# phylo42/EPIK

Measured on AMD Instinct MI355X. Metric: reads placed/sec, higher is better.
Workload: dtype f32

## Files before the change

epik_amd/capi.py:

```python
from __future__ import annotations

import ctypes
import os

import numpy as np

_HERE = os.path.dirname(os.path.abspath(__file__))
LIB_PATH = os.environ.get("EPIK_AMD_LIB") or os.path.join(_HERE, "libepik_amd.so")

ABI_VERSION = 3

OK, ERR_INVALID, ERR_NO_DEVICE, ERR_HIP, ERR_UNSUPPORTED = 0, 1, 2, 3, 4

PLACEMENT = np.dtype([("branch", np.uint32), ("score", np.float32), ("lwr", np.float64)])
CONFIDENCE = np.dtype([("clade", np.uint32), ("clade_mass_q", np.uint32), ("edpl", np.float64)])
TAXON_RECORD = np.dtype([("taxon", np.uint32), ("taxon_mass_q", np.uint32), ("first_taxon", np.uint32), ("total_q", np.uint32)])
WINDOW_RECORD = np.dtype([("call", np.uint32), ("call_mass_q", np.uint32), ("first_group", np.uint32), ("total_q", np.uint32)])
WINDOW_SEGMENT = np.dtype([("call", np.uint32), ("first_window", np.uint32), ("num_windows", np.uint32), ("reserved", np.uint32),
                           ("call_mass", np.uint64), ("total", np.uint64)])
TAXA_TOTALS = np.dtype([(name, np.uint64) for name in ("placed", "no_hit", "too_short", "too_narrow", "no_mass", "bad_reads")])
SQUASH_MERGE = np.dtype([("a", np.uint32), ("b", np.uint32), ("dist", np.float64), ("len_a", np.float64), ("len_b", np.float64)])
SQUASH_NONE = 0xFFFFFFFF
EPCA_INFO = np.dtype([("used", np.uint32), ("components", np.uint32), ("sweeps", np.uint32), ("converged", np.uint32),
                      ("trace", np.float64), ("scale", np.float64)])
# ... 71 lines not shown
RAREFY_MAX_DEPTHS = 256
RAREFY_MAX_DEPTH = 1 << 20
PKDB_VALUE = np.dtype([("branch", np.uint32), ("score", np.float32)])

EXPORTS = (
    "epik_amd_device_count",
    "epik_amd_last_error",
    "epik_amd_placer_create",
    "epik_amd_placer_plan",
    "epik_amd_placer_plan_sizes",
    "epik_amd_placer_build_image",
    "epik_amd_placer_plan_run_counts",
    "epik_amd_placer_run_counts",
    "epik_amd_placer_ring_form",
    "epik_amd_placer_table_form",
    "epik_amd_placer_destroy",
    "epik_amd_placer_place",
    "epik_amd_placer_place_device",
    "epik_amd_placer_algorithmic_bytes",
    "epik_amd_placer_create_sharded",
    "epik_amd_placer_accumulate_device",
    "epik_amd_placer_finish_device",
    "epik_amd_placer_partial_info",
    "epik_amd_placer_accumulate_lists_device",
    "epik_amd_placer_finish_lists_device",
    "epik_amd_placer_last_path",
    "epik_amd_placer_stream_build",
    "epik_amd_placer_place_sharded",
    "epik_amd_placer_release_scratch",
    "epik_amd_placer_set_wide_counts",
# ... 263 lines not shown
    0xFFFFFFFF, 0xFFFFFFFE, 0xFFFFFFFD, 0xFFFFFFFC, 0xFFFFFFFB, 0xFFFFFFFA)
WINDOW_CLASSES = {WINDOW_TOO_NARROW: "too_narrow", WINDOW_TOO_SHORT: "too_short", WINDOW_NO_HIT: "no_hit",
                  WINDOW_BAD_ROW: "bad_row", WINDOW_NO_MASS: "no_mass", WINDOW_AMBIGUOUS: "ambiguous"}

STRAND_FORWARD, STRAND_REVERSE, STRAND_BOTH = 0, 1, 2
STRANDS = {"forward": STRAND_FORWARD, "reverse": STRAND_REVERSE, "both": STRAND_BOTH}

MATES_FF = 0x100
MATE_ORIENTATIONS = {"fr": 0, "ff": MATES_FF}

FRAMES_FORWARD, FRAMES_REVERSE, FRAMES_BOTH = 0, 1, 2
FRAME_MODES = {"forward": FRAMES_FORWARD, "reverse": FRAMES_REVERSE, "both": FRAMES_BOTH}
FRAME_NAMES = ("+1", "+2", "+3", "-1", "-2", "-3")

ROWS_COUNTS_TOO_NARROW = 0xFFFFFFFF


class EpikAmdError(RuntimeError):
    def __init__(self, code: int, message: str):
        super().__init__(f"libepik_amd error {code}: {message}")
        self.code = code


_lib = None


def hip_runtimes(maps_text: str | None = None) -> list:
    import re
    if maps_text is None:
        try:
# ... 62 lines not shown
    lib.epik_amd_placer_plan_sizes.restype = i32
    lib.epik_amd_placer_plan_sizes.argtypes = [ctypes.c_uint32] * 4 + [ctypes.POINTER(ListBin), u64, ctypes.c_uint32, ctypes.c_uint32,
                                               u64, ctypes.POINTER(Plan)]
    lib.epik_amd_placer_build_image.restype = i32
    lib.epik_amd_placer_build_image.argtypes = [ctypes.POINTER(PlacerDesc), ctypes.c_uint32, ctypes.c_uint32, u64,
                                                vp, vp, vp]
    lib.epik_amd_placer_plan_run_counts.restype = i32
    lib.epik_amd_placer_plan_run_counts.argtypes = [ctypes.POINTER(PlacerDesc), ctypes.c_uint32, ctypes.c_uint32, u64,
                                                    ctypes.c_uint32, ctypes.POINTER(ctypes.c_uint32)]
    lib.epik_amd_placer_run_counts.restype = i32
    lib.epik_amd_placer_run_counts.argtypes = [vp, ctypes.c_uint32, ctypes.POINTER(ctypes.c_uint32)]
    lib.epik_amd_placer_ring_form.restype = i32
    lib.epik_amd_placer_ring_form.argtypes = [vp, ctypes.c_uint32, ctypes.POINTER(ctypes.c_uint32)]
    lib.epik_amd_placer_table_form.restype = i32
    lib.epik_amd_placer_table_form.argtypes = [vp, ctypes.POINTER(ctypes.c_uint32)]
    lib.epik_amd_placer_destroy.restype = None
    lib.epik_amd_placer_destroy.argtypes = [vp]
    lib.epik_amd_placer_place.restype = i32
    lib.epik_amd_placer_place.argtypes = [vp, vp, vp, u64, vp, vp, vp]
    lib.epik_amd_placer_place_device.restype = i32
    lib.epik_amd_placer_place_device.argtypes = [vp, vp, vp, u64, vp, vp, vp, vp]
    lib.epik_amd_placer_algorithmic_bytes.restype = i32
    lib.epik_amd_placer_algorithmic_bytes.argtypes = [vp, vp, vp, u64, vp, vp, ctypes.POINTER(u64)]
    lib.epik_amd_placer_launch_info.restype = i32
    lib.epik_amd_placer_launch_info.argtypes = [vp, ctypes.POINTER(ctypes.c_uint32),
                                                ctypes.POINTER(ctypes.c_uint32),
                                                ctypes.POINTER(ctypes.c_uint32)]
    lib.epik_amd_placer_set_wide_counts.restype = i32
    lib.epik_amd_placer_set_wide_counts.argtypes = [vp, i32]
    lib.epik_amd_placer_choose_counts.restype = i32
# ... 296 lines not shown
```

epik_amd/csrc/capi.hip:

```cpp
#include <hip/hip_runtime.h>

#include <algorithm>
#include <atomic>
#include <cmath>
#include <cstdio>
#include <cstdlib>
#include <cstring>
#include <new>
#include <string>
#include <thread>
#include <vector>

#include "db_image.hpp"
#include "epik_amd.h"
#include "place_kernel.h"
#include "placer_impl.hpp"

namespace {

thread_local std::string g_last_error;

int fail(int code, const std::string &msg)
{
    g_last_error = msg;
// ... 95 lines not shown
        (void)hipFree(p->params.dbg);
    }
#endif
    (void)hipFree(p->d_table);
    (void)hipFree(p->d_filter);
    (void)hipFree(p->d_postings);
    (void)hipFree(p->d_char_class);
    (void)hipFree(p->d_seqs);
    (void)hipFree(p->d_seq_offsets);
    (void)hipFree(p->d_rows);
    (void)hipFree(p->d_n_rows);
    (void)hipFree(p->d_counts);
    (void)hipFree(p->d_total);
    (void)hipFree(p->d_front_hdr);
    (void)hipFree(p->d_finish_hdr);
    (void)hipFree(p->d_slow_list);
    (void)hipFree(p->d_slice_rows);
    (void)hipFree(p->d_slice_sums);
    (void)hipFree(p->d_front_pool);
    (void)hipFree(p->d_front_cursor);
    (void)hipFree(p->d_sparse_cap);
    (void)hipFree(p->d_scan_tiles);
    if (p->h_front_cursor) (void)hipHostFree(p->h_front_cursor);
    if (p->ev_start) (void)hipEventDestroy(p->ev_start);
    if (p->ev_stop) (void)hipEventDestroy(p->ev_stop);
    for (hipEvent_t e : p->ev_in) (void)hipEventDestroy(e);
    for (hipEvent_t e : p->ev_kernel) (void)hipEventDestroy(e);
    if (p->stream) (void)hipStreamDestroy(p->stream);
    if (p->stream_in) (void)hipStreamDestroy(p->stream_in);
    if (p->stream_out) (void)hipStreamDestroy(p->stream_out);
// ... 143 lines not shown
    CREATE_TRY(hipMemGetInfo(&free_mem, &total_mem));
    const image::Source src{d, shard_index, shard_count};
    image::Plan &plan = p->plan;
    if (const int rc = image::make_plan(src, free_mem, std::getenv("EPIK_AMD_LAYOUT"), std::getenv("EPIK_AMD_KERNEL"),
                                        plan, err);
        rc != EPIK_AMD_OK) {
        return fail(rc, err);
    }
    p->layout = plan.layout;
    p->team = plan.layout == epik_amd::DbLayout::kTeam;
    const bool run_lists = image::run_counts_apply(plan, std::getenv("EPIK_AMD_RUN_COUNTS"));
    p->runs = run_lists ? epik_amd::kRunLists : plan.runs ? epik_amd::kRunsMixed : 0;
    {
        const char *form = std::getenv("EPIK_AMD_RING_FORM");
        p->ring_near = p->runs != 0 && plan.posting_bytes < epik_amd::kNearRegionBytes && !(form && std::strcmp(form, "far") == 0);
    }
    p->db_bytes = plan.posting_bytes;
    CREATE_TRY(hipStreamCreateWithFlags(&p->stream, hipStreamNonBlocking));
    CREATE_TRY(hipStreamCreateWithFlags(&p->stream_in, hipStreamNonBlocking));
    CREATE_TRY(hipStreamCreateWithFlags(&p->stream_out, hipStreamNonBlocking));
    CREATE_TRY(hipMalloc(&p->d_table, plan.table_bytes));
    if (plan.filter_bytes) CREATE_TRY(hipMalloc(reinterpret_cast<void **>(&p->d_filter), plan.filter_bytes));
    CREATE_TRY(hipMalloc(reinterpret_cast<void **>(&p->d_postings), plan.posting_bytes));
    {
        DeviceSink table, filter, postings;
        CREATE_TRY(table.init(static_cast<uint8_t *>(p->d_table), plan.table_bytes, p->stream_in));
        if (plan.filter_bytes)
            CREATE_TRY(filter.init(reinterpret_cast<uint8_t *>(p->d_filter), plan.filter_bytes, p->stream_out));
        CREATE_TRY(postings.init(p->d_postings, plan.posting_bytes, p->stream));
        const int rc = image::build(src, plan, table, plan.filter_bytes ? &filter : nullptr, postings, err);
// ... 25 lines not shown
    pp.filter_rec_bytes = plan.filter_rec_bytes;
    pp.entry_len_bits = plan.len_bits;
    pp.entry_cell_bits = plan.cell_bits;
    pp.postings = p->d_postings;
    pp.char_class = p->d_char_class;
    pp.sigma_pow_km1 = (uint32_t)(d->num_keys / d->alphabet_size);
    pp.kmer_size = d->kmer_size;
    pp.alphabet_size = d->alphabet_size;
    pp.num_branches = d->num_branches;
    pp.keep_at_most = d->keep_at_most;
    pp.keep_factor = d->keep_factor;
    pp.threshold = d->threshold;
    pp.log_threshold = d->log_threshold;
#ifdef EPIK_AMD_ABLATION
    if (const char *ab = std::getenv("EPIK_AMD_ABLATE")) pp.ablate = (uint32_t)std::atoi(ab);
    if (const char *e = std::getenv("EPIK_AMD_GRID_PERCENT")) p->grid_percent = std::strtoull(e, nullptr, 10);
    if (const char *st = std::getenv("EPIK_AMD_STAMPS"); st && st[0] == '1') {
        CREATE_TRY(hipMalloc(reinterpret_cast<void **>(&pp.dbg), kDbgWords * sizeof(unsigned long long)));
        CREATE_TRY(hipMemset(pp.dbg, 0, kDbgWords * sizeof(unsigned long long)));
    }
#endif
    hipDeviceProp_t prop;
    CREATE_TRY(hipGetDeviceProperties(&prop, d->device));
    if (p->team) {
        p->team_waves = plan.team_waves;
        p->team_table = static_cast<const uint8_t *>(p->d_table);
        p->team_passes = plan.team_passes;
        p->team_slice_rows = plan.team_slice_rows;
        p->team_rows_pad = plan.team_rows_pad;
        const uint32_t desc_bytes = epik_amd::team_desc_bytes(d->keep_at_most);
// ... 74 lines not shown
            const int runs = p->runs | g.ring;
            if (counts == epik_amd::kCounts8 && (pp.n_pad + 7u) / 8u > desc_bytes) {
                g.max_blocks = 0;
                continue;
            }
            if (g.lds_wave_bytes > kMaxLdsPerBlock) {
                return fail(EPIK_AMD_ERR_UNSUPPORTED, "num_branches too large for the one-wavefront-per-read kernel");
            }
            uint32_t best_waves = 0;
            for (uint32_t wpb = 4; wpb >= 1; wpb >>= 1) {
                const uint32_t block_bytes = wpb * g.lds_wave_bytes;
                if (block_bytes > kMaxLdsPerBlock) continue;
                CREATE_TRY(epik_amd::set_place_reads_lds_limit(p->layout, runs, counts, block_bytes));
                int per_cu = 0;
                CREATE_TRY(epik_amd::place_reads_occupancy(p->layout, runs, counts, (int)(wpb * 64u), block_bytes, &per_cu));
                const uint32_t lds_units = (block_bytes + epik_amd::kLdsGranule - 1u) / epik_amd::kLdsGranule;
                per_cu = std::min<int>(per_cu, (int)(128u / std::max(lds_units, 1u)));
                if (per_cu < 1) per_cu = 1;
                if ((uint32_t)per_cu * wpb > best_waves) {
                    best_waves = (uint32_t)per_cu * wpb;
                    g.waves_per_block = wpb;
                    g.lds_block_bytes = block_bytes;
                    g.max_blocks = (uint32_t)prop.multiProcessorCount * (uint32_t)per_cu;
                }
            }
            g.resident_waves = best_waves;
            CREATE_TRY(epik_amd::set_place_reads_lds_limit(p->layout, runs, counts, g.lds_block_bytes));
            CREATE_TRY(epik_amd::set_finish_reads_lds_limit(counts, g.lds_block_bytes));
        }
    }
// ... 258 lines not shown
            if (asked > est) est = asked;
        }
        want = (uint64_t)est + 1024u;
        size_t free_b = 0, total_b = 0;
        if (hipMemGetInfo(&free_b, &total_b) == hipSuccess) {
            const uint64_t room = ((uint64_t)free_b + p->front_pool_cap * 8u) / 2u / 8u;
            want = std::min<uint64_t>(want, std::max<uint64_t>(room, 1024u));
        }
    }
    want = (want + 7u) & ~7ull;
    if (want > p->front_pool_cap || (p->front_pool_forced && want != p->front_pool_cap)) {
        (void)hipFree(p->d_front_pool);
        p->d_front_pool = nullptr, p->front_pool_cap = 0;
        HIP_TRY(hipMalloc(reinterpret_cast<void **>(&p->d_front_pool), (size_t)want * sizeof(uint64_t)));
        p->front_pool_cap = want;
    }
    return EPIK_AMD_OK;
}

static int launch(epik_amd_placer *p, launch_mode mode, const void *d_seqs, const void *d_seq_offsets, uint64_t n,
                  void *d_rows, void *d_n_rows, void *d_counts, hipStream_t stream, const shard_buffers &shard = {},
                  uint64_t total_chars = 0)
{
    if (n == 0) return EPIK_AMD_OK;
    const bool lists = mode == kAccumulateLists || mode == kFinishLists;
    epik_amd::PlaceParams pp = p->params;
    pp.partial_scores = shard.scores;
    pp.partial_counts = shard.counts;
    pp.max_kmers_cap = (mode == kAccumulate || mode == kFinish) ? 65535u : 0u;
    pp.amb_slot = shard.amb_slot;
// ... 104 lines not shown
                tp.read_list = p->d_slow_list;
                tp.read_list_count = p->d_front_cursor + 1;
                HIP_TRY(epik_amd::launch_team(tp, p->team_waves, p->counts, (int)mode, dim3((unsigned)blocks),
                                              g.lds_block_bytes, stream));
                HIP_TRY(hipMemcpyAsync(p->h_front_cursor, p->d_front_cursor, 3 * sizeof(unsigned long long),
                                       hipMemcpyDeviceToHost, stream));
            }
        } else {
            HIP_TRY(epik_amd::launch_team(tp, p->team_waves, p->counts, (int)mode, dim3((unsigned)blocks), g.lds_block_bytes,
                                          stream));
        }
    } else if (mode == kFinish) {
        HIP_TRY(epik_amd::launch_finish_reads(pp, p->counts, dim3((unsigned)blocks), dim3(g.waves_per_block * 64u),
                                              g.lds_block_bytes, stream));
    } else {
        HIP_TRY(epik_amd::launch_place_reads(pp, p->layout, p->runs | p->geo[p->counts].ring, p->counts, dim3((unsigned)blocks),
                                             dim3(g.waves_per_block * 64u), g.lds_block_bytes, stream));
    }
    if (timed) {
        HIP_TRY(hipEventRecord(p->ev_stop, stream));
        p->ev_recorded = true;
    }
    return EPIK_AMD_OK;
}

int epik_amd_placer_accumulate_device(epik_amd_placer *p, const void *d_seqs, const void *d_seq_offsets,
                                      uint64_t n, void *d_scores, void *d_counts, const void *d_amb_slot,
                                      void *d_amb_order, void *d_amb_avg, void *stream)
{
    if (!p) return fail(EPIK_AMD_ERR_INVALID, "null placer");
    if (n && (!d_seqs || !d_seq_offsets || !d_scores || !d_counts))
        return fail(EPIK_AMD_ERR_INVALID, "null device buffer");
// ... 120 lines not shown

int epik_amd_placer_run_counts(const epik_amd_placer *p, uint32_t counts, uint32_t *lists)
{
    if (!p || !lists) return fail(EPIK_AMD_ERR_INVALID, "null argument");
    if (counts > (uint32_t)epik_amd::kCounts32) return fail(EPIK_AMD_ERR_INVALID, "counts must be 0, 1 or 2");
    *lists = !p->team && p->runs == epik_amd::kRunLists && counts != (uint32_t)epik_amd::kCounts8;
    return EPIK_AMD_OK;
}

int epik_amd_placer_ring_form(const epik_amd_placer *p, uint32_t counts, uint32_t *form)
{
    if (!p || !form) return fail(EPIK_AMD_ERR_INVALID, "null argument");
    if (counts > (uint32_t)epik_amd::kCounts32) return fail(EPIK_AMD_ERR_INVALID, "counts must be 0, 1 or 2");
    const int ring = p->team ? 0 : p->geo[counts].ring;
    *form = ((ring & epik_amd::kRingNear) ? EPIK_AMD_RING_NEAR : 0u) | ((ring & epik_amd::kRingSlack) ? EPIK_AMD_RING_SLACK : 0u);
    return EPIK_AMD_OK;
}

int epik_amd_placer_table_form(const epik_amd_placer *p, uint32_t *form)
{
    if (!p || !form) return fail(EPIK_AMD_ERR_INVALID, "null argument");
    switch (p->layout) {
        case epik_amd::DbLayout::kPacked:
        case epik_amd::DbLayout::kFiltered: *form = EPIK_AMD_TABLE_BY_CODE; break;
        case epik_amd::DbLayout::kPaired: *form = EPIK_AMD_TABLE_PAIRED; break;
        case epik_amd::DbLayout::kTripled: *form = EPIK_AMD_TABLE_TRIPLED; break;
        default: *form = 0u;
    }
    return EPIK_AMD_OK;
}
// ... 213 lines not shown
    return EPIK_AMD_OK;
}

int epik_amd_placer_release_scratch(epik_amd_placer *p)
{
    if (!p) return fail(EPIK_AMD_ERR_INVALID, "null placer");
    HIP_TRY(hipSetDevice(p->device));
    HIP_TRY(hipDeviceSynchronize());
    if (p->shard_state && p->shard_state_free) p->shard_state_free(p->shard_state);
    p->shard_state = nullptr;
    void **bufs[] = {reinterpret_cast<void **>(&p->d_front_hdr), reinterpret_cast<void **>(&p->d_finish_hdr),
                     reinterpret_cast<void **>(&p->d_slow_list), &p->d_slice_rows,
                     &p->d_slice_sums, reinterpret_cast<void **>(&p->d_front_pool), reinterpret_cast<void **>(&p->d_sparse_cap),
                     reinterpret_cast<void **>(&p->d_scan_tiles), reinterpret_cast<void **>(&p->d_seqs),
                     reinterpret_cast<void **>(&p->d_seq_offsets), reinterpret_cast<void **>(&p->d_rows),
                     reinterpret_cast<void **>(&p->d_n_rows), reinterpret_cast<void **>(&p->d_counts)};
    for (void **b : bufs) {
        if (*b) (void)hipFree(*b);
        *b = nullptr;
    }
    p->front_hdr_bytes = 0, p->finish_hdr_bytes = 0, p->slow_list_reads = 0, p->slice_out_reads = 0, p->front_pool_cap = 0, p->sparse_cap_items = 0;
    p->d_seqs_cap = 0, p->d_reads_cap = 0, p->front_failed_reads = 0;
    return EPIK_AMD_OK;
}

int epik_amd_placer_launch_info(const epik_amd_placer *p, uint32_t *waves_per_block,
                                uint32_t *blocks, uint32_t *lds_bytes)
{
    if (!p) return fail(EPIK_AMD_ERR_INVALID, "null placer");
    const auto &g = p->geo[p->last_geo];
    const bool streaming = p->team && p->team_front && p->last_streamed;
    if (waves_per_block) *waves_per_block = streaming ? (uint32_t)g.stream_bw[g.last_stream] : g.waves_per_block;
    if (blocks) *blocks = p->last_blocks ? p->last_blocks : streaming ? g.stream_blocks[g.last_stream] : g.max_blocks;
    if (lds_bytes) *lds_bytes = streaming ? g.stream_lds_bytes[g.last_stream] : g.lds_block_bytes;
    return EPIK_AMD_OK;
}

// ... 39 lines not shown
```

epik_amd/csrc/place_device.hpp:

```cpp
#ifndef EPIK_AMD_PLACE_DEVICE_HPP
#define EPIK_AMD_PLACE_DEVICE_HPP
#include <hip/hip_runtime.h>
#include <float.h>
#include <stdint.h>

#include <type_traits>

#include "place_kernel.h"

namespace epik_amd {

namespace {

constexpr int kWave = 64;
constexpr int kTilesPerPass = EPIK_AMD_TILES_PER_PASS;
constexpr int kRing = EPIK_AMD_RING;
static_assert((kRing & (kRing - 1)) == 0 && kRing >= 4 && kRing <= 32, "kRing: power of two, one descriptor lane per stage");
constexpr uint32_t kChunkCap = (uint32_t)kTilesPerPass * 64u;

typedef unsigned int v2u __attribute__((ext_vector_type(2)));
typedef unsigned int v4u __attribute__((ext_vector_type(4)));
typedef int v4i __attribute__((ext_vector_type(4)));

__device__ __forceinline__ int lane_id() { return (int)__lane_id(); }
// ... 420 lines not shown
                         "v_min_u32 %1, %5, %1"
                         : "=&v"(score), "=&v"(addr)
                         : "v"(lane4), "s"(srd), "s"(base), "s"(score_top), "n"(kSettled ? 1 : 0)
                         : "memory");
        }
    }
};
template <typename Layout, typename = void>
struct SlackBytes : std::integral_constant<uint32_t, 0u> {};
template <typename Layout>
struct SlackBytes<Layout, std::void_t<decltype(Layout::kSlackBytes)>> : std::integral_constant<uint32_t, Layout::kSlackBytes> {};
template <typename Layout, typename = void>
struct ListCounts : std::false_type {};
template <typename Layout>
struct ListCounts<Layout, std::void_t<decltype(Layout::kListCounts)>> : std::bool_constant<Layout::kListCounts> {};

template <typename Layout>
__device__ __forceinline__ uint64_t chunk_address(const PlaceParams &p, uint64_t addr, uint32_t c)
{
    return (uint64_t)(p.postings + addr + (uint64_t)c * Layout::kChunkBytes);
}
__device__ __forceinline__ uint64_t null_chunk(const PlaceParams &p) { return (uint64_t)p.postings; }

__device__ __forceinline__ uint32_t tile_char(const uint8_t *__restrict__ seq, uint64_t len, uint64_t tile_pos)
{
    const uint64_t pos = tile_pos + (uint64_t)lane_id();
    return seq[pos < len ? pos : len - 1];
}
__device__ __forceinline__ uint32_t tile_class(uint32_t ch, uint64_t len, uint64_t tile_pos,
                                               const uint32_t *__restrict__ char_class)
// ... 357 lines not shown
                v[q] = (uint32_t)s;
            }
        }
        const uint32_t incl = wave_incl_scan_u32((uint32_t)s);
        const uint32_t front = carry + incl - (uint32_t)s;
        const uint32_t add = sizeof(CountT) == 2 ? front * 0x10001u : front;
        if (mine) {
#pragma unroll
            for (uint32_t q = 0; q < kVecs; ++q)
                at[q] = v4u{v[4 * q] + add, v[4 * q + 1] + add, v[4 * q + 2] + add, v[4 * q + 3] + add};
        }
        carry += __builtin_amdgcn_readlane(incl, 63);
    }
}

struct WaveCtx {
    static constexpr bool kTeam = false;
    static constexpr uint32_t kCandCap = kChunkCap;
    __device__ __forceinline__ bool untouched() const { return false; }
    template <typename Params>
    __device__ __forceinline__ uint32_t rows_pad(const Params &p) const { return p.n_pad; }
    template <typename Params>
    __device__ __forceinline__ uint32_t rows(const Params &p) const { return p.num_branches; }
    __device__ __forceinline__ uint32_t branch_base() const { return 0u; }
    __device__ __forceinline__ uint32_t kmer_size(const PlaceParams &p) const { return p.kmer_size; }
    __device__ __forceinline__ float log_threshold(const PlaceParams &p) const { return p.log_threshold; }
    __device__ __forceinline__ uint32_t keep_at_most(const PlaceParams &p) const { return p.keep_at_most; }
    template <typename Layout>
    __device__ __forceinline__ void lookup(const PlaceParams &p, uint32_t key, uint64_t &addr, uint32_t &len) const
    {
        Layout::lookup(p, key, 0u, addr, len);
    }
};

template <typename Layout, typename CountT, typename Ctx>
__device__ __attribute__((noinline)) void place_ambiguous(const PlaceParams *__restrict__ kp, WaveLds<CountT> lds,
                                                          const uint8_t *__restrict__ seq, uint64_t len,
                                                          uint64_t n_kmers, int64_t amb_slot, Ctx ctx)
{
    const PlaceParams &p = *kp;
    const int lane = lane_id();
    const uint32_t k = p.kmer_size;
    const uint32_t sigma = p.alphabet_size;
    const uint32_t stride = kWave - (k - 1);
    const float k_f = (float)k;
    const uint32_t rows_pad = ctx.rows_pad(p);
    auto *seen_bitmap = reinterpret_cast<typename WaveLds<CountT>::u32_t *>(lds.desc);
    if (sizeof(CountT) == 1)
// ... 64 lines not shown
                    }
                }
            }
        }
    }
}

struct TeamPartial {
    uint32_t touched;
    uint32_t relative;
    float ref_score;
    uint32_t reserved;
    double sum;
};

#ifndef EPIK_AMD_TAU_STOP
#define EPIK_AMD_TAU_STOP 8
#endif
template <typename Layout, typename CountT, typename Ctx>
__device__ __forceinline__ void place_epilogue_body(const PlaceParams *__restrict__ kp, WaveLds<CountT> lds,
                                                    uint64_t read, uint64_t n_kmers, Ctx ctx)
{
    const PlaceParams &p = *kp;
    const int lane = lane_id();
#ifdef EPIK_AMD_ABLATION
#define EPI_STAMP(k)                                                                   \
    if constexpr (Ctx::kTeam) {                                                        \
        if (ctx.trace_at_ != 0xffffffffu && lane == 0) {                               \
            const uint32_t i_ = ctx.trace_at_ + ((k) == 10 ? 0u : (uint32_t)(k) + 1u); \
            if (i_ < 100000u) {                                                        \
// ... 310 lines not shown
                ctx.cand[my_rank[q]] = v4u{(uint32_t)(my_key[q] >> 32), ctx.branch_base() + row,
                                           (uint32_t)lds.count[row] & ~(uint32_t)lds.kSeen, 0u};
            }
        }
        for (uint32_t r = n_sel + (uint32_t)lane; r < keep; r += kWave) ctx.cand[r] = v4u{0u, 0u, 0u, 0u};
        if (lane == 0) {
            ctx.partial->touched = touched;
            ctx.partial->relative = relative_sum ? 1u : 0u;
            ctx.partial->ref_score = ref_score;
            ctx.partial->sum = sum;
        }
        EPI_STAMP(6)
        if (!untouched) lds.clear(n_rows_pad);
        EPI_STAMP(7)
        (void)read;
        return;
    }
    double my_power[kQ];
    double best_power = 0.0;
#pragma unroll
    for (int q = 0; q < kQ; ++q) {
        my_power[q] = 0.0;
        if ((uint32_t)q < n_q) {
            const bool has_row = my_key[q] != 0 && my_rank[q] < n_sel;
            if (has_row && !all_underflow) my_power[q] = pow10_f64((double)unord_f32((uint32_t)(my_key[q] >> 32)));
            const uint64_t first = __ballot(has_row && my_rank[q] == 0);
            if (first)
                best_power = __longlong_as_double(
                    (long long)readlane_u64((uint64_t)__double_as_longlong(my_power[q]), __builtin_ctzll(first)));
        }
// ... 128 lines not shown
```

epik_amd/csrc/place_kernel.h:

```cpp
#ifndef EPIK_AMD_PLACE_KERNEL_H
#define EPIK_AMD_PLACE_KERNEL_H

#include <hip/hip_runtime.h>
#include <stdint.h>

#include "epik_amd.h"

#include "db_layout.h"

namespace epik_amd {

struct PlaceParams {
    const void *table;
    const uint64_t *filter;
    uint32_t sigma_pow_km1;
    uint32_t filter_rec_bytes;
    const uint8_t *postings;
    const uint32_t *char_class;
    const uint8_t *seqs;
    const uint64_t *seq_offsets;
    uint64_t n_reads;
    epik_amd_placement *rows;
    uint32_t *n_rows;
    uint32_t *kmer_counts;
    float *partial_scores;
    uint16_t *partial_counts;
    const int32_t *amb_slot;
    uint32_t *amb_order;
    float *amb_avg;
    uint32_t kmer_size;
    uint32_t alphabet_size;
    uint32_t num_branches;
    uint32_t keep_at_most;
    double keep_factor;
    float threshold;
    float log_threshold;
    uint32_t max_kmers_cap;
    uint32_t n_pad;
    uint32_t lds_wave_bytes;
    uint32_t entry_len_bits;
    uint32_t entry_cell_bits;
    uint32_t ablate;
    unsigned long long *dbg;
};

constexpr uint32_t kCountsTooNarrow = 0xffffffffu;

struct TeamParams {
    PlaceParams base;
    const uint8_t *team_table;
    uint64_t num_keys;
    uint32_t shard_index, shard_count;
    uint32_t team_paired;
    uint32_t passes;
    uint32_t slice_rows;
    uint32_t rows_pad;
    uint32_t desc_cap;
    uint32_t slice_bytes;
    uint32_t desc_bytes;
// ... 48 lines not shown
uint64_t sparse_scan_tiles(uint64_t part_reads, uint32_t slices);
hipError_t launch_team_sparse_scan(const TeamParams &tp, int waves, unsigned long long *tile_sums, hipStream_t stream);
hipError_t launch_team_headers(const TeamParams &tp, int waves, int counts, hipStream_t stream);
hipError_t launch_team_merge(const TeamParams &tp, int waves, dim3 grid, hipStream_t stream);
constexpr size_t kTeamPartialBytes = 24;
hipError_t set_team_stream_lds_limit(int waves, int counts, int mode, int bw, size_t lds_bytes);
bool team_stream_is_wide(int waves, size_t lds_bytes, int bw);
hipError_t team_stream_occupancy(int waves, int counts, int mode, int bw, size_t lds_bytes, int *blocks_per_cu);
hipError_t launch_team_algorithmic_bytes(const TeamParams &tp, int waves, unsigned long long *d_total, hipStream_t stream);

enum : int { kRunsMixed = 1, kRunLists = 2, kRingNear = 4, kRingSlack = 8 };
hipError_t launch_place_reads(const PlaceParams &p, DbLayout layout, int runs, int counts, dim3 grid, dim3 block,
                              size_t lds_bytes, hipStream_t stream);
hipError_t set_place_reads_lds_limit(DbLayout layout, int runs, int counts, size_t lds_bytes);
hipError_t place_reads_occupancy(DbLayout layout, int runs, int counts, int block_threads, size_t lds_bytes,
                                 int *blocks_per_cu);
hipError_t launch_finish_reads(const PlaceParams &p, int counts, dim3 grid, dim3 block, size_t lds_bytes,
                               hipStream_t stream);
hipError_t set_finish_reads_lds_limit(int counts, size_t lds_bytes);
hipError_t launch_algorithmic_bytes(const PlaceParams &p, DbLayout layout, int runs, unsigned long long *d_total,
                                    hipStream_t stream);

}
#endif
```

epik_amd/csrc/place_kernel.hip:

```cpp
#include <hip/hip_runtime.h>
#include <stdint.h>

#include <type_traits>

#include "place_device.hpp"

namespace epik_amd {

template <typename Layout, typename CountT>
__global__ __launch_bounds__(256, 5) void place_reads_kernel(PlaceParams p)
{
    extern __shared__ __align__(16) unsigned char lds_raw[];
    const int lane = lane_id();
    const uint32_t wave_in_block = __builtin_amdgcn_readfirstlane(threadIdx.x >> 6);
    const uint32_t waves_per_block = blockDim.x >> 6;

    WaveLds<CountT> lds;
    {
        unsigned char *base = lds_raw + (size_t)wave_in_block * p.lds_wave_bytes;
        lds.carve(base, p.n_pad, SlackBytes<Layout>::value);
    }
    const uint32_t score_row0 = __builtin_amdgcn_readfirstlane((uint32_t)(uintptr_t)lds.score);
    const uint32_t score_top = __builtin_amdgcn_readfirstlane((uint32_t)(uintptr_t)lds.score + (p.n_pad - 1u) * 4u);
    const uint32_t count_top = __builtin_amdgcn_readfirstlane((uint32_t)(uintptr_t)lds.count +
// ... 23 lines not shown
#else
#define EPIK_STAMP(k)
#endif
    for (uint64_t read = wave_global; read < p.n_reads; read += total_waves) {
        const uint64_t seq_begin = readlane_u64(p.seq_offsets[read], 0);
        const uint64_t len = readlane_u64(p.seq_offsets[read + 1], 0) - seq_begin;
        const uint8_t *__restrict__ seq = p.seqs + seq_begin;
        if (len < k || len - k + 1 > WaveLds<CountT>::kMaxKmers || (p.max_kmers_cap && len - k + 1 > p.max_kmers_cap)) {
            if (p.partial_scores) {
                for (uint32_t i = lane; i < p.num_branches; i += kWave) {
                    p.partial_scores[read * p.num_branches + i] = 0.0f;
                    p.partial_counts[read * p.num_branches + i] = 0u;
                }
            } else if (lane == 0) {
                p.n_rows[read] = len < k ? 0u : kCountsTooNarrow;
            }
            continue;
        }
        const uint64_t n_kmers = len - k + 1;
        bool any_amb = false;

        for (uint64_t pass_pos = 0; pass_pos < n_kmers; pass_pos += (uint64_t)kTilesPerPass * stride) {
            uint64_t start[kTilesPerPass];
            uint32_t llen[kTilesPerPass];
            uint32_t tile_cls[kTilesPerPass];
#pragma unroll
            for (int t = 0; t < kTilesPerPass; ++t) tile_cls[t] = tile_char(seq, len, pass_pos + (uint64_t)t * stride);
#pragma unroll
            for (int t = 0; t < kTilesPerPass; ++t)
                tile_cls[t] = tile_class(tile_cls[t], len, pass_pos + (uint64_t)t * stride, p.char_class);
// ... 109 lines not shown
            continue;
        }
#endif
        if (p.partial_scores) {
            for (uint32_t i = lane; i < p.n_pad; i += kWave) {
                const uint2 cv = lds.load(i);
                if (i < p.num_branches) {
                    p.partial_scores[read * p.num_branches + i] = __uint_as_float(cv.x);
                    p.partial_counts[read * p.num_branches + i] = (uint16_t)(cv.y & ~(uint32_t)WaveLds<CountT>::kSeen);
                }
                lds.store(i, 0u, 0u);
            }
            continue;
        }
        if (lane == 0) lds.store(p.n_pad - 1u, 0u, 0u);
        place_epilogue<Layout, CountT>(kp, lds, read, n_kmers, WaveCtx{});
        EPIK_STAMP(4)
    }
#ifdef EPIK_AMD_ABLATION
    if (p.dbg && lane == 0)
        for (int i = 0; i < 8; ++i) atomicAdd(&p.dbg[i], dbg_t[i]);
#endif
}

template <typename CountT>
__global__ __launch_bounds__(256, 5) void finish_reads_kernel(PlaceParams p)
{
    extern __shared__ __align__(16) unsigned char lds_raw[];
    const int lane = lane_id();
    const uint32_t wave_in_block = __builtin_amdgcn_readfirstlane(threadIdx.x >> 6);
    const uint32_t waves_per_block = blockDim.x >> 6;
// ... 99 lines not shown
    }
    return hipErrorInvalidValue;
}

}

hipError_t launch_place_reads(const PlaceParams &p, DbLayout layout, int runs, int counts, dim3 grid, dim3 block,
                              size_t lds_bytes, hipStream_t stream)
{
    return dispatch(layout, runs, counts, [&]<typename L, typename C>() {
        hipLaunchKernelGGL((place_reads_kernel<L, C>), grid, block, lds_bytes, stream, p);
        return hipGetLastError();
    });
}

hipError_t set_place_reads_lds_limit(DbLayout layout, int runs, int counts, size_t )
{
    return dispatch(layout, runs, counts, [&]<typename L, typename C>() {
        return hipFuncSetAttribute(reinterpret_cast<const void *>(&place_reads_kernel<L, C>),
                                   hipFuncAttributeMaxDynamicSharedMemorySize, (int)kLdsPerCu);
    });
}

hipError_t place_reads_occupancy(DbLayout layout, int runs, int counts, int block_threads, size_t lds_bytes,
                                 int *blocks_per_cu)
{
    return dispatch(layout, runs, counts, [&]<typename L, typename C>() {
        return hipOccupancyMaxActiveBlocksPerMultiprocessor(blocks_per_cu, place_reads_kernel<L, C>,
                                                            block_threads, lds_bytes);
    });
}

hipError_t launch_finish_reads(const PlaceParams &p, int counts, dim3 grid, dim3 block, size_t lds_bytes,
                               hipStream_t stream)
{
    return dispatch_counts<PackedLayout<kPlainTable>>(counts, [&]<typename L, typename C>() {
        hipLaunchKernelGGL((finish_reads_kernel<C>), grid, block, lds_bytes, stream, p);
        return hipGetLastError();
    });
}

hipError_t set_finish_reads_lds_limit(int counts, size_t )
// ... 21 lines not shown
```

epik_amd/csrc/placer_impl.hpp:

```cpp
#ifndef EPIK_AMD_PLACER_IMPL_HPP
#define EPIK_AMD_PLACER_IMPL_HPP
#include <hip/hip_runtime.h>

#include <string>
#include <vector>

#include "db_image.hpp"
#include "epik_amd.h"
#include "place_kernel.h"

struct epik_amd_placer {
    int device = 0;
    epik_amd::DbLayout layout = epik_amd::DbLayout::kCompact32;
    int counts = epik_amd::kCounts16;
    bool counts_forced = false;
    bool timing = false;
    void *d_table = nullptr;
    uint64_t *d_filter = nullptr;
    uint8_t *d_postings = nullptr;
    uint64_t db_bytes = 0;
    uint32_t *d_char_class = nullptr;
    uint64_t generation = 0;
    void *shard_state = nullptr;
    void (*shard_state_free)(void *) = nullptr;
    std::vector<uint32_t> h_char_class;
    epik_amd::PlaceParams params{};
    epik_amd::image::Plan plan{};
    int runs = 0;
    bool ring_near = false;
    bool team = false;
    int team_waves = 0;
    const uint8_t *team_table = nullptr;
    uint32_t team_passes = 0, team_slice_rows = 0, team_rows_pad = 0;
    bool team_front = false;
    uint8_t *d_front_hdr = nullptr;
    size_t front_hdr_bytes = 0;
    uint8_t *d_finish_hdr = nullptr;
    size_t finish_hdr_bytes = 0;
    uint64_t *d_slow_list = nullptr;
    size_t slow_list_reads = 0;
    void *d_slice_rows = nullptr, *d_slice_sums = nullptr;
    size_t slice_out_reads = 0;
    uint64_t *d_front_pool = nullptr;
    uint64_t front_pool_cap = 0;
// ... 49 lines not shown
```

epik_amd/provenance.py:

```python
from __future__ import annotations

import hashlib
import os

ROOT = os.path.dirname(os.path.dirname(os.path.abspath(__file__)))
KERNEL_SOURCES = ("place_kernel.hip", "place_device.hpp", "team_kernel.hip", "team_stream.hip", "team_device.hpp",
                  "team_epilogue.hpp", "place_kernel.h", "db_layout.h", "db_image.cpp", "capi.hip", "placer_impl.hpp")


def kernel_source_hash() -> str:
    h = hashlib.sha256()
    for name in KERNEL_SOURCES:
        with open(os.path.join(ROOT, "epik_amd", "csrc", name), "rb") as fh:
            h.update(name.encode() + b"\0" + fh.read())
    return h.hexdigest()[:16]


def built_with() -> dict:
    import json
    try:
        with open(os.path.join(ROOT, "epik_amd", "libepik_amd.build.json")) as fh:
            return json.load(fh)
    except (OSError, ValueError):
        return {}
# ... 32 lines not shown
```

include/epik_amd.h:

```cpp
#ifndef EPIK_AMD_H
#define EPIK_AMD_H

#include <stddef.h>
#include <stdint.h>

#ifdef __cplusplus
extern "C" {
#endif

#define EPIK_AMD_ABI_VERSION 3

enum epik_amd_status {
    EPIK_AMD_OK = 0,
    EPIK_AMD_ERR_INVALID = 1,
    EPIK_AMD_ERR_NO_DEVICE = 2,
    EPIK_AMD_ERR_HIP = 3,
    EPIK_AMD_ERR_UNSUPPORTED = 4
};

typedef struct {
    uint32_t branch;
    float score;
} epik_amd_pkdb_value;

// ... 54 lines not shown
    uint64_t lists_in_runs;
} epik_amd_list_bin;
int epik_amd_placer_plan_sizes(uint32_t kmer_size, uint32_t alphabet_size, uint32_t num_branches, uint32_t keep_at_most,
                               const epik_amd_list_bin *bins, uint64_t n_bins, uint32_t shard_index, uint32_t shard_count,
                               uint64_t free_bytes, epik_amd_plan *plan);
int epik_amd_placer_plan_run_counts(const epik_amd_placer_desc *desc, uint32_t shard_index, uint32_t shard_count,
                                    uint64_t free_bytes, uint32_t counts, uint32_t *lists);
int epik_amd_placer_run_counts(const epik_amd_placer *p, uint32_t counts, uint32_t *lists);
#define EPIK_AMD_RING_NEAR 1u
#define EPIK_AMD_RING_SLACK 2u
int epik_amd_placer_ring_form(const epik_amd_placer *p, uint32_t counts, uint32_t *form);
#define EPIK_AMD_TABLE_BY_CODE 1u
#define EPIK_AMD_TABLE_PAIRED 2u
#define EPIK_AMD_TABLE_TRIPLED 3u
int epik_amd_placer_table_form(const epik_amd_placer *p, uint32_t *form);
int epik_amd_placer_build_image(const epik_amd_placer_desc *desc, uint32_t shard_index, uint32_t shard_count,
                                uint64_t free_bytes, void *table, void *filter, void *postings);

void epik_amd_placer_destroy(epik_amd_placer *p);

int epik_amd_placer_place(epik_amd_placer *p, const char *seqs, const uint64_t *seq_offsets,
                          uint64_t n, epik_amd_placement *rows, uint32_t *n_rows,
                          uint32_t *kmer_counts);

int epik_amd_placer_place_device(epik_amd_placer *p, const void *d_seqs, const void *d_seq_offsets,
                                 uint64_t n, void *d_rows, void *d_n_rows, void *d_kmer_counts,
                                 void *stream);

int epik_amd_placer_algorithmic_bytes(epik_amd_placer *p, const void *d_seqs,
                                      const void *d_seq_offsets, uint64_t n, const void *d_n_rows,
// ... 750 lines not shown
```

Baseline: 218.3 million.

## Defer per-read LWR tail to a separate finish-rows kernel

The placement kernel no longer computes powers, LWR ratios and the keep-factor filter in its wave epilogue. It writes a per-read header (sum, ref/threshold scores, flags) and the selected candidates to a workspace, and a second lightweight kernel spreads each read's candidates across a lane group to finish the LWR and compaction. The aim is to cut register pressure and serial double-precision work in the heavy LDS-bound kernel, which could raise occupancy. The cost is an extra kernel launch plus a round trip of workspace traffic through global memory.

New measurement: 221.0 million, median of 6. +1.2%, better.

```diff
diff --git a/epik_amd/capi.py b/epik_amd/capi.py
--- a/epik_amd/capi.py
+++ b/epik_amd/capi.py
@@ -109,6 +109,7 @@
     "epik_amd_placer_run_counts",
     "epik_amd_placer_ring_form",
     "epik_amd_placer_table_form",
+    "epik_amd_placer_tail_form",
     "epik_amd_placer_destroy",
     "epik_amd_placer_place",
     "epik_amd_placer_place_device",
@@ -402,6 +403,7 @@
 FRAME_NAMES = ("+1", "+2", "+3", "-1", "-2", "-3")
 
 ROWS_COUNTS_TOO_NARROW = 0xFFFFFFFF
+TAIL_WAVE, TAIL_KERNEL = 0, 1
 
 
 class EpikAmdError(RuntimeError):
@@ -494,6 +496,9 @@
     lib.epik_amd_placer_ring_form.argtypes = [vp, ctypes.c_uint32, ctypes.POINTER(ctypes.c_uint32)]
     lib.epik_amd_placer_table_form.restype = i32
     lib.epik_amd_placer_table_form.argtypes = [vp, ctypes.POINTER(ctypes.c_uint32)]
+    if hasattr(lib, "epik_amd_placer_tail_form"):
+        lib.epik_amd_placer_tail_form.restype = i32
+        lib.epik_amd_placer_tail_form.argtypes = [vp, ctypes.c_uint32, ctypes.POINTER(ctypes.c_uint32)]
     lib.epik_amd_placer_destroy.restype = None
     lib.epik_amd_placer_destroy.argtypes = [vp]
     lib.epik_amd_placer_place.restype = i32
diff --git a/epik_amd/csrc/capi.hip b/epik_amd/csrc/capi.hip
--- a/epik_amd/csrc/capi.hip
+++ b/epik_amd/csrc/capi.hip
@@ -133,6 +133,7 @@
     (void)hipFree(p->d_total);
     (void)hipFree(p->d_front_hdr);
     (void)hipFree(p->d_finish_hdr);
+    (void)hipFree(p->d_tail_ws);
     (void)hipFree(p->d_slow_list);
     (void)hipFree(p->d_slice_rows);
     (void)hipFree(p->d_slice_sums);
@@ -306,6 +307,9 @@
     {
         const char *form = std::getenv("EPIK_AMD_RING_FORM");
         p->ring_near = p->runs != 0 && plan.posting_bytes < epik_amd::kNearRegionBytes && !(form && std::strcmp(form, "far") == 0);
+        const char *tail = std::getenv("EPIK_AMD_TAIL");
+        p->tail_kernel = !p->team && p->runs == epik_amd::kRunLists && d->keep_at_most >= 1 &&
+                         d->keep_at_most <= epik_amd::kTailMaxKeep && !(tail && std::strcmp(tail, "wave") == 0);
     }
     p->db_bytes = plan.posting_bytes;
     CREATE_TRY(hipStreamCreateWithFlags(&p->stream, hipStreamNonBlocking));
@@ -361,6 +365,7 @@
     pp.log_threshold = d->log_threshold;
 #ifdef EPIK_AMD_ABLATION
     if (const char *ab = std::getenv("EPIK_AMD_ABLATE")) pp.ablate = (uint32_t)std::atoi(ab);
+    if (pp.ablate) p->tail_kernel = false;
     if (const char *e = std::getenv("EPIK_AMD_GRID_PERCENT")) p->grid_percent = std::strtoull(e, nullptr, 10);
     if (const char *st = std::getenv("EPIK_AMD_STAMPS"); st && st[0] == '1') {
         CREATE_TRY(hipMalloc(reinterpret_cast<void **>(&pp.dbg), kDbgWords * sizeof(unsigned long long)));
@@ -465,6 +470,11 @@
                 CREATE_TRY(epik_amd::set_place_reads_lds_limit(p->layout, runs, counts, block_bytes));
                 int per_cu = 0;
                 CREATE_TRY(epik_amd::place_reads_occupancy(p->layout, runs, counts, (int)(wpb * 64u), block_bytes, &per_cu));
+                if (p->tail_kernel && counts != epik_amd::kCounts8) {
+                    int deferred = 0;
+                    CREATE_TRY(epik_amd::place_reads_occupancy(p->layout, runs, counts, (int)(wpb * 64u), block_bytes, &deferred, true));
+                    per_cu = std::min(per_cu, deferred);
+                }
                 const uint32_t lds_units = (block_bytes + epik_amd::kLdsGranule - 1u) / epik_amd::kLdsGranule;
                 per_cu = std::min<int>(per_cu, (int)(128u / std::max(lds_units, 1u)));
                 if (per_cu < 1) per_cu = 1;
@@ -753,6 +763,18 @@
         p->d_front_pool = nullptr, p->front_pool_cap = 0;
         HIP_TRY(hipMalloc(reinterpret_cast<void **>(&p->d_front_pool), (size_t)want * sizeof(uint64_t)));
         p->front_pool_cap = want;
+    }
+    return EPIK_AMD_OK;
+}
+
+static int reserve_tail(epik_amd_placer *p, uint64_t n)
+{
+    if (epik_amd::tail_ws_bytes(n, p->params.keep_at_most) > p->tail_ws_bytes) {
+        const size_t bytes = epik_amd::tail_ws_bytes(n + n / 4 + 64, p->params.keep_at_most);
+        (void)hipFree(p->d_tail_ws);
+        p->d_tail_ws = nullptr, p->tail_ws_bytes = 0;
+        HIP_TRY(hipMalloc(reinterpret_cast<void **>(&p->d_tail_ws), bytes));
+        p->tail_ws_bytes = bytes;
     }
     return EPIK_AMD_OK;
 }
@@ -887,8 +909,16 @@
         HIP_TRY(epik_amd::launch_finish_reads(pp, p->counts, dim3((unsigned)blocks), dim3(g.waves_per_block * 64u),
                                               g.lds_block_bytes, stream));
     } else {
-        HIP_TRY(epik_amd::launch_place_reads(pp, p->layout, p->runs | p->geo[p->counts].ring, p->counts, dim3((unsigned)blocks),
-                                             dim3(g.waves_per_block * 64u), g.lds_block_bytes, stream));
+        const bool deferred = mode == kPlace && p->tail_kernel && p->counts != epik_amd::kCounts8;
+        if (deferred) {
+            if (const int rc = reserve_tail(p, n); rc != EPIK_AMD_OK) return rc;
+            HIP_TRY(epik_amd::launch_place_reads_deferred(pp, p->d_tail_ws, p->layout, p->runs | p->geo[p->counts].ring, p->counts,
+                                                          dim3((unsigned)blocks), dim3(g.waves_per_block * 64u), g.lds_block_bytes, stream));
+            HIP_TRY(epik_amd::launch_finish_rows(pp, p->d_tail_ws, stream));
+        } else {
+            HIP_TRY(epik_amd::launch_place_reads(pp, p->layout, p->runs | p->geo[p->counts].ring, p->counts, dim3((unsigned)blocks),
+                                                 dim3(g.waves_per_block * 64u), g.lds_block_bytes, stream));
+        }
     }
     if (timed) {
         HIP_TRY(hipEventRecord(p->ev_stop, stream));
@@ -1039,6 +1069,14 @@
     if (counts > (uint32_t)epik_amd::kCounts32) return fail(EPIK_AMD_ERR_INVALID, "counts must be 0, 1 or 2");
     const int ring = p->team ? 0 : p->geo[counts].ring;
     *form = ((ring & epik_amd::kRingNear) ? EPIK_AMD_RING_NEAR : 0u) | ((ring & epik_amd::kRingSlack) ? EPIK_AMD_RING_SLACK : 0u);
+    return EPIK_AMD_OK;
+}
+
+int epik_amd_placer_tail_form(const epik_amd_placer *p, uint32_t counts, uint32_t *form)
+{
+    if (!p || !form) return fail(EPIK_AMD_ERR_INVALID, "null argument");
+    if (counts > (uint32_t)epik_amd::kCounts32) return fail(EPIK_AMD_ERR_INVALID, "counts must be 0, 1 or 2");
+    *form = p->tail_kernel && counts != (uint32_t)epik_amd::kCounts8 ? EPIK_AMD_TAIL_KERNEL : EPIK_AMD_TAIL_WAVE;
     return EPIK_AMD_OK;
 }
 
@@ -1282,13 +1320,14 @@
                      &p->d_slice_sums, reinterpret_cast<void **>(&p->d_front_pool), reinterpret_cast<void **>(&p->d_sparse_cap),
                      reinterpret_cast<void **>(&p->d_scan_tiles), reinterpret_cast<void **>(&p->d_seqs),
                      reinterpret_cast<void **>(&p->d_seq_offsets), reinterpret_cast<void **>(&p->d_rows),
-                     reinterpret_cast<void **>(&p->d_n_rows), reinterpret_cast<void **>(&p->d_counts)};
+                     reinterpret_cast<void **>(&p->d_n_rows), reinterpret_cast<void **>(&p->d_counts),
+                     reinterpret_cast<void **>(&p->d_tail_ws)};
     for (void **b : bufs) {
         if (*b) (void)hipFree(*b);
         *b = nullptr;
     }
     p->front_hdr_bytes = 0, p->finish_hdr_bytes = 0, p->slow_list_reads = 0, p->slice_out_reads = 0, p->front_pool_cap = 0, p->sparse_cap_items = 0;
-    p->d_seqs_cap = 0, p->d_reads_cap = 0, p->front_failed_reads = 0;
+    p->d_seqs_cap = 0, p->d_reads_cap = 0, p->front_failed_reads = 0, p->tail_ws_bytes = 0;
     return EPIK_AMD_OK;
 }
 
diff --git a/epik_amd/csrc/place_device.hpp b/epik_amd/csrc/place_device.hpp
--- a/epik_amd/csrc/place_device.hpp
+++ b/epik_amd/csrc/place_device.hpp
@@ -458,6 +458,14 @@
 struct ListCounts : std::false_type {};
 template <typename Layout>
 struct ListCounts<Layout, std::void_t<decltype(Layout::kListCounts)>> : std::bool_constant<Layout::kListCounts> {};
+template <typename Layout>
+struct DeferredTail : Layout {
+    static constexpr bool kDeferTail = true;
+};
+template <typename Layout, typename = void>
+struct DefersTail : std::false_type {};
+template <typename Layout>
+struct DefersTail<Layout, std::void_t<decltype(Layout::kDeferTail)>> : std::bool_constant<Layout::kDeferTail> {};
 
 template <typename Layout>
 __device__ __forceinline__ uint64_t chunk_address(const PlaceParams &p, uint64_t addr, uint32_t c)
@@ -845,8 +853,10 @@
     }
 }
 
-struct WaveCtx {
+template <bool kDeferTailT>
+struct WaveCtxT {
     static constexpr bool kTeam = false;
+    static constexpr bool kDeferTail = kDeferTailT;
     static constexpr uint32_t kCandCap = kChunkCap;
     __device__ __forceinline__ bool untouched() const { return false; }
     template <typename Params>
@@ -863,6 +873,9 @@
         Layout::lookup(p, key, 0u, addr, len);
     }
 };
+typedef WaveCtxT<false> WaveCtx;
+template <typename Ctx>
+constexpr bool kDefersTail = requires { requires Ctx::kDeferTail; };
 
 template <typename Layout, typename CountT, typename Ctx>
 __device__ __attribute__((noinline)) void place_ambiguous(const PlaceParams *__restrict__ kp, WaveLds<CountT> lds,
@@ -957,6 +970,21 @@
     double sum;
 };
 
+struct alignas(16) TailHeader {
+    double sum;
+    float ref_score;
+    float thr_score;
+    float not_placed;
+    uint32_t bits;
+    uint32_t reserved[2];
+};
+static_assert(sizeof(TailHeader) == kTailHeaderBytes && sizeof(v4u) == kTailRowBytes, "the workspace the host sizes (place_kernel.h)");
+constexpr uint32_t kTailSelMask = 0xffu;
+constexpr uint32_t kTailRelative = 0x100u;
+constexpr uint32_t kTailUnderflow = 0x200u;
+constexpr uint32_t kTailUntouched = 0x400u;
+constexpr uint32_t kTailNone = 0x800u;
+
 #ifndef EPIK_AMD_TAU_STOP
 #define EPIK_AMD_TAU_STOP 8
 #endif
@@ -1297,6 +1325,50 @@
         if (!untouched) lds.clear(n_rows_pad);
         EPI_STAMP(7)
         (void)read;
+        return;
+    }
+    if constexpr (kDefersTail<Ctx>) {
+        const float not_placed = (float)N - (float)touched;
+        double sum;
+        if (relative_sum) {
+            sum = wave_sum_f64((double)rel_sum);
+            if (not_placed != 0.0f)
+                sum += (double)(not_placed *
+                                __builtin_amdgcn_exp2f(__fmul_rn(__fsub_rn(thr_score, ref_score), kLog2Of10)));
+        } else {
+            sum = 0.0;
+            if (!all_underflow) {
+                for (uint32_t i = lane; i < N; i += kWave) {
+                    const uint2 cv = lds.load(i);
+                    if (cv.y != 0) sum += pow10_f64((double)__uint_as_float(cv.x));
+                }
+                sum = wave_sum_f64(sum);
+            }
+        }
+        TailHeader *headers = static_cast<TailHeader *>(p.tail_ws);
+        TailHeader *hdr = headers + read;
+        v4u *rows_out = reinterpret_cast<v4u *>(headers + p.n_reads) + read * keep;
+#pragma unroll
+        for (int q = 0; q < kQ; ++q) {
+            if ((uint32_t)q < n_q && my_key[q] != 0 && my_rank[q] < n_sel) {
+                const uint32_t branch = ~(uint32_t)my_key[q];
+                uint32_t count = 0u;
+                if (p.kmer_counts) count = (touched && branch < N) ? ((uint32_t)lds.count[branch] & ~(uint32_t)lds.kSeen) : 0u;
+                rows_out[my_rank[q]] = v4u{branch, __float_as_uint(unord_f32((uint32_t)(my_key[q] >> 32))), count, 0u};
+            }
+        }
+        if (lane == 0) {
+            TailHeader h;
+            h.sum = sum;
+            h.ref_score = ref_score;
+            h.thr_score = thr_score;
+            h.not_placed = not_placed;
+            h.bits = n_sel | (relative_sum ? kTailRelative : 0u) | (all_underflow ? kTailUnderflow : 0u) |
+                     (touched == 0 ? kTailUntouched : 0u);
+            h.reserved[0] = h.reserved[1] = 0u;
+            *hdr = h;
+        }
+        lds.clear(n_rows_pad);
         return;
     }
     double my_power[kQ];
diff --git a/epik_amd/csrc/place_kernel.h b/epik_amd/csrc/place_kernel.h
--- a/epik_amd/csrc/place_kernel.h
+++ b/epik_amd/csrc/place_kernel.h
@@ -24,7 +24,10 @@
     uint32_t *n_rows;
     uint32_t *kmer_counts;
     float *partial_scores;
-    uint16_t *partial_counts;
+    union {
+        uint16_t *partial_counts;
+        void *tail_ws;
+    };
     const int32_t *amb_slot;
     uint32_t *amb_order;
     float *amb_avg;
@@ -43,6 +46,9 @@
     uint32_t ablate;
     unsigned long long *dbg;
 };
+constexpr size_t kTailHeaderBytes = 32, kTailRowBytes = 16;
+constexpr size_t tail_ws_bytes(uint64_t n_reads, uint32_t keep) { return (size_t)n_reads * (kTailHeaderBytes + (size_t)keep * kTailRowBytes); }
+constexpr uint32_t kTailMaxKeep = 64;
 
 constexpr uint32_t kCountsTooNarrow = 0xffffffffu;
 
@@ -121,7 +127,10 @@
                               size_t lds_bytes, hipStream_t stream);
 hipError_t set_place_reads_lds_limit(DbLayout layout, int runs, int counts, size_t lds_bytes);
 hipError_t place_reads_occupancy(DbLayout layout, int runs, int counts, int block_threads, size_t lds_bytes,
-                                 int *blocks_per_cu);
+                                 int *blocks_per_cu, bool deferred_tail = false);
+hipError_t launch_place_reads_deferred(const PlaceParams &p, void *tail_ws, DbLayout layout, int runs, int counts, dim3 grid,
+                                       dim3 block, size_t lds_bytes, hipStream_t stream);
+hipError_t launch_finish_rows(const PlaceParams &p, void *tail_ws, hipStream_t stream);
 hipError_t launch_finish_reads(const PlaceParams &p, int counts, dim3 grid, dim3 block, size_t lds_bytes,
                                hipStream_t stream);
 hipError_t set_finish_reads_lds_limit(int counts, size_t lds_bytes);
diff --git a/epik_amd/csrc/place_kernel.hip b/epik_amd/csrc/place_kernel.hip
--- a/epik_amd/csrc/place_kernel.hip
+++ b/epik_amd/csrc/place_kernel.hip
@@ -61,6 +61,7 @@
                 }
             } else if (lane == 0) {
                 p.n_rows[read] = len < k ? 0u : kCountsTooNarrow;
+                if constexpr (DefersTail<Layout>::value) static_cast<TailHeader *>(p.tail_ws)[read].bits = kTailNone;
             }
             continue;
         }
@@ -200,7 +201,7 @@
             continue;
         }
         if (lane == 0) lds.store(p.n_pad - 1u, 0u, 0u);
-        place_epilogue<Layout, CountT>(kp, lds, read, n_kmers, WaveCtx{});
+        place_epilogue<Layout, CountT>(kp, lds, read, n_kmers, WaveCtxT<DefersTail<Layout>::value>{});
         EPIK_STAMP(4)
     }
 #ifdef EPIK_AMD_ABLATION
@@ -330,18 +331,44 @@
     });
 }
 
+hipError_t launch_place_reads_deferred(const PlaceParams &p, void *tail_ws, DbLayout layout, int runs, int counts, dim3 grid,
+                                       dim3 block, size_t lds_bytes, hipStream_t stream)
+{
+    if (!tail_ws || p.partial_scores) return hipErrorInvalidValue;
+    PlaceParams q = p;
+    q.tail_ws = tail_ws;
+    return dispatch(layout, runs, counts, [&]<typename L, typename C>() {
+        if constexpr (ListCounts<L>::value) {
+            hipLaunchKernelGGL((place_reads_kernel<DeferredTail<L>, C>), grid, block, lds_bytes, stream, q);
+            return hipGetLastError();
+        } else {
+            return hipErrorInvalidValue;
+        }
+    });
+}
+
 hipError_t set_place_reads_lds_limit(DbLayout layout, int runs, int counts, size_t )
 {
     return dispatch(layout, runs, counts, [&]<typename L, typename C>() {
+        if constexpr (ListCounts<L>::value) {
+            const hipError_t e = hipFuncSetAttribute(reinterpret_cast<const void *>(&place_reads_kernel<DeferredTail<L>, C>),
+                                                     hipFuncAttributeMaxDynamicSharedMemorySize, (int)kLdsPerCu);
+            if (e != hipSuccess) return e;
+        }
         return hipFuncSetAttribute(reinterpret_cast<const void *>(&place_reads_kernel<L, C>),
                                    hipFuncAttributeMaxDynamicSharedMemorySize, (int)kLdsPerCu);
     });
 }
 
 hipError_t place_reads_occupancy(DbLayout layout, int runs, int counts, int block_threads, size_t lds_bytes,
-                                 int *blocks_per_cu)
+                                 int *blocks_per_cu, bool deferred_tail)
 {
     return dispatch(layout, runs, counts, [&]<typename L, typename C>() {
+        if constexpr (ListCounts<L>::value) {
+            if (deferred_tail)
+                return hipOccupancyMaxActiveBlocksPerMultiprocessor(blocks_per_cu, place_reads_kernel<DeferredTail<L>, C>,
+                                                                    block_threads, lds_bytes);
+        }
         return hipOccupancyMaxActiveBlocksPerMultiprocessor(blocks_per_cu, place_reads_kernel<L, C>,
                                                             block_threads, lds_bytes);
     });
diff --git a/epik_amd/csrc/placer_impl.hpp b/epik_amd/csrc/placer_impl.hpp
--- a/epik_amd/csrc/placer_impl.hpp
+++ b/epik_amd/csrc/placer_impl.hpp
@@ -28,6 +28,9 @@
     epik_amd::image::Plan plan{};
     int runs = 0;
     bool ring_near = false;
+    bool tail_kernel = false;
+    uint8_t *d_tail_ws = nullptr;
+    size_t tail_ws_bytes = 0;
     bool team = false;
     int team_waves = 0;
     const uint8_t *team_table = nullptr;
diff --git a/epik_amd/csrc/tail_device.hpp b/epik_amd/csrc/tail_device.hpp
--- /dev/null
+++ b/epik_amd/csrc/tail_device.hpp
@@ -0,0 +1,71 @@
+#ifndef EPIK_AMD_TAIL_DEVICE_HPP
+#define EPIK_AMD_TAIL_DEVICE_HPP
+#include "place_device.hpp"
+
+namespace epik_amd {
+namespace {
+
+template <uint32_t kGroup>
+__device__ __forceinline__ void finish_rows_group(const PlaceParams &p, const void *tail_ws, uint64_t read, uint32_t r, bool active)
+{
+    static_assert(kGroup >= 1 && kGroup <= 64 && (kGroup & (kGroup - 1u)) == 0, "a power of two of lanes inside a wave");
+    const uint32_t lane = (uint32_t)lane_id();
+    const uint32_t group_at = lane & ~(kGroup - 1u);
+    const uint32_t keep = p.keep_at_most;
+    const TailHeader *headers = static_cast<const TailHeader *>(tail_ws);
+    const v4u *cands = reinterpret_cast<const v4u *>(headers + p.n_reads);
+    TailHeader h{};
+    h.bits = active ? headers[read].bits : kTailNone;
+    const bool none = (h.bits & kTailNone) != 0;
+    if (!none) h = headers[read];
+    const uint32_t n_sel = none ? 0u : (h.bits & kTailSelMask);
+    const bool has_row = r < n_sel && r < keep;
+    v4u cand{0u, 0u, 0u, 0u};
+    if (has_row) cand = cands[read * keep + r];
+    const bool all_underflow = (h.bits & kTailUnderflow) != 0;
+    const float score = __uint_as_float(cand.y);
+    double my_power = 0.0;
+    if (has_row && !all_underflow) my_power = pow10_f64((double)score);
+    double best_power = my_power;
+    float best_score = score;
+    if constexpr (kGroup > 1) {
+        const uint64_t bits = (uint64_t)__double_as_longlong(my_power);
+        const uint32_t lo = (uint32_t)__shfl((int)(uint32_t)bits, (int)group_at);
+        const uint32_t hi = (uint32_t)__shfl((int)(uint32_t)(bits >> 32), (int)group_at);
+        best_power = __longlong_as_double((long long)(((uint64_t)hi << 32) | lo));
+        best_score = __uint_as_float((uint32_t)__shfl((int)cand.y, (int)group_at));
+    }
+    double score_sum;
+    if (h.bits & kTailRelative) {
+        const double rel = h.sum;
+        const double ref_power = (h.ref_score == best_score) ? best_power : pow10_f64((double)h.ref_score);
+        score_sum = ref_power * rel;
+    } else {
+        const double sum_placed = h.sum;
+        score_sum = all_underflow ? 0.0 : (double)h.not_placed * pow10_f64((double)h.thr_score) + sum_placed;
+    }
+    const double keep_factor = (score_sum == 0.0) ? 0.0 : p.keep_factor;
+
+    const double best_ratio =
+        (score_sum == 0.0 || best_power == 0.0) ? 0.0 : best_power / score_sum;
+    const double ratio_threshold = best_ratio * keep_factor;
+    double my_lwr = 0.0;
+    if (has_row && score_sum != 0.0 && my_power != 0.0) my_lwr = my_power / score_sum;
+    const bool kept = has_row && my_lwr >= ratio_threshold;
+    const uint64_t group_mask = kGroup == 64 ? ~0ull : (((1ull << kGroup) - 1ull) << group_at);
+    const uint64_t kept_ranks = __ballot(kept) & group_mask;
+    if (kept) {
+        const uint32_t slot = (uint32_t)__popcll(kept_ranks & ((1ull << lane) - 1ull));
+        epik_amd_placement out;
+        out.branch = cand.x;
+        out.score = score;
+        out.lwr = my_lwr;
+        p.rows[read * keep + slot] = out;
+        if (p.kmer_counts) p.kmer_counts[read * keep + slot] = cand.z;
+    }
+    if (active && !none && r == 0) p.n_rows[read] = (uint32_t)__popcll(kept_ranks);
+}
+
+}
+}
+#endif
diff --git a/epik_amd/csrc/tail_kernel.hip b/epik_amd/csrc/tail_kernel.hip
--- /dev/null
+++ b/epik_amd/csrc/tail_kernel.hip
@@ -0,0 +1,47 @@
+#include <hip/hip_runtime.h>
+#include <stdint.h>
+
+#include "tail_device.hpp"
+
+namespace epik_amd {
+
+constexpr uint32_t kTailBlock = 256;
+
+template <uint32_t kGroup>
+__global__ __launch_bounds__(kTailBlock) void finish_rows_kernel(PlaceParams p)
+{
+    const uint64_t thread = (uint64_t)blockIdx.x * kTailBlock + threadIdx.x;
+    const uint64_t read = thread / kGroup;
+    finish_rows_group<kGroup>(p, p.tail_ws, read, (uint32_t)(thread % kGroup), read < p.n_reads);
+}
+
+namespace {
+
+template <uint32_t kGroup>
+hipError_t launch_group(const PlaceParams &p, void *tail_ws, hipStream_t stream)
+{
+    PlaceParams q = p;
+    q.tail_ws = tail_ws;
+    const uint64_t blocks = (p.n_reads * kGroup + kTailBlock - 1u) / kTailBlock;
+    if (blocks > 0x7fffffffull) return hipErrorInvalidValue;
+    hipLaunchKernelGGL((finish_rows_kernel<kGroup>), dim3((unsigned)blocks), dim3(kTailBlock), 0, stream, q);
+    return hipGetLastError();
+}
+
+}
+
+hipError_t launch_finish_rows(const PlaceParams &p, void *tail_ws, hipStream_t stream)
+{
+    if (!tail_ws || p.keep_at_most == 0 || p.keep_at_most > kTailMaxKeep) return hipErrorInvalidValue;
+    if (p.n_reads == 0) return hipSuccess;
+    const uint32_t keep = p.keep_at_most;
+    if (keep <= 1) return launch_group<1>(p, tail_ws, stream);
+    if (keep <= 2) return launch_group<2>(p, tail_ws, stream);
+    if (keep <= 4) return launch_group<4>(p, tail_ws, stream);
+    if (keep <= 8) return launch_group<8>(p, tail_ws, stream);
+    if (keep <= 16) return launch_group<16>(p, tail_ws, stream);
+    if (keep <= 32) return launch_group<32>(p, tail_ws, stream);
+    return launch_group<64>(p, tail_ws, stream);
+}
+
+}
diff --git a/epik_amd/provenance.py b/epik_amd/provenance.py
--- a/epik_amd/provenance.py
+++ b/epik_amd/provenance.py
@@ -5,7 +5,7 @@
 
 ROOT = os.path.dirname(os.path.dirname(os.path.abspath(__file__)))
 KERNEL_SOURCES = ("place_kernel.hip", "place_device.hpp", "team_kernel.hip", "team_stream.hip", "team_device.hpp",
-                  "team_epilogue.hpp", "place_kernel.h", "db_layout.h", "db_image.cpp", "capi.hip", "placer_impl.hpp")
+                  "team_epilogue.hpp", "tail_kernel.hip", "tail_device.hpp", "place_kernel.h", "db_layout.h", "db_image.cpp", "capi.hip", "placer_impl.hpp")
 
 
 def kernel_source_hash() -> str:
diff --git a/include/epik_amd.h b/include/epik_amd.h
--- a/include/epik_amd.h
+++ b/include/epik_amd.h
@@ -92,6 +92,9 @@
 #define EPIK_AMD_TABLE_PAIRED 2u
 #define EPIK_AMD_TABLE_TRIPLED 3u
 int epik_amd_placer_table_form(const epik_amd_placer *p, uint32_t *form);
+#define EPIK_AMD_TAIL_WAVE 0u
+#define EPIK_AMD_TAIL_KERNEL 1u
+int epik_amd_placer_tail_form(const epik_amd_placer *p, uint32_t counts, uint32_t *form);
 int epik_amd_placer_build_image(const epik_amd_placer_desc *desc, uint32_t shard_index, uint32_t shard_count,
                                 uint64_t free_bytes, void *table, void *filter, void *postings);
 
```
